# menmitsu/opticalFlowClustering

Measured on AMD Instinct MI355X. Metric: Mpixels/s dense flow+kmeans @1080p, higher is better.
Workload: dtype f32 storage, f64 accumulation; 1 GPU; BASELINE.json configs[2]: 300-frame 1080p synthetic clip, Farneback flow (0.5,3,15,3,5,1.2,0) + Lloyd k=5 over (u,v), frames sharded over 1 GPU(s); width=1920, height=1080, frames=300, pairs=299, k=5, lloyd_iters=11, flow_batch_pairs=64

## Files before the change

### include/ofc.h

```cpp
#ifndef OFC_H
#define OFC_H
#include <stddef.h>
#include <stdint.h>

#ifdef __cplusplus
extern "C" {
#endif

#define OFC_VERSION 100

enum {
    OFC_OK = 0,
    OFC_EINVAL = -1,
    OFC_ENODEV = -2,
    OFC_EHIP = -3,
    OFC_ENOMEM = -4,
    OFC_ENOTREADY = -5,
    OFC_EUNSUPPORTED = -6,
    OFC_ECOMM = -7
};

enum { OFC_U8 = 0, OFC_F32 = 1, OFC_F64 = 2 };

int ofc_version(void);
// ... 67 lines not shown
int ofc_grid_cell_means(int device, const uint8_t *bgr, int W, int H, int rows, int cols,
                        uint8_t *mean_bgr, uint8_t *hsv);

int ofc_kmeans_fit(int device, const void *X, int dtype, int64_t N, int d, int k,
                   const double *init, int max_iter, double tol_rel, double *centers,
                   int32_t *labels, double *inertia, int *n_iter);
int ofc_kmeans_predict(int device, const void *X, int dtype, int64_t N, int d, int k,
                       const double *centers, int32_t *labels);
int ofc_kmeans_fit_dev(int device, const void *X_dev, int dtype, int64_t N, int d, int k,
                       const double *init, int max_iter, double tol_rel, double *centers,
                       uint8_t *labels_dev, double *inertia, int *n_iter);
int ofc_kmeans_fit_dev_stats(int device, const void *X_dev, int dtype, int64_t N, int d, int k,
                             const double *init, int max_iter, double tol_rel, const double *colsum,
                             double *centers, uint8_t *labels_dev, double *inertia, int *n_iter);
int ofc_lloyd_prune_stats(int device, double *out6);
int ofc_bench_lloyd_sweep(int device, const float *X_dev, int64_t N, int k, const double *centers, const double *mean,
                          int what, int iters, float *ms_per_launch);
int ofc_lloyd_colstats_dev(int device, const void *X_dev, int dtype, int64_t N, int d, const double *mean,
                           int pass, double *out);
int ofc_lloyd_step_dev(int device, const void *X_dev, int dtype, int64_t N, int d, int k, const double *mean,
                       const double *centers_c, uint8_t *labels_dev, int accumulate, double *record);
int ofc_lloyd_inertia_dev(int device, const void *X_dev, int dtype, int64_t N, int d, int k, const double *mean,
                          const double *centers_c, const uint8_t *labels_dev, double *inertia);
int ofc_lloyd_farthest_dev(int device, const void *X_dev, int dtype, int64_t N, int d, int k, const double *mean,
                           const double *centers_c, const uint8_t *labels_dev, const int64_t *excl, int n_excl,
                           double *dist2, int64_t *index, double *x_c, int *label);

int ofc_kmeans_fit_w(int device, const void *X, int dtype, const void *w, int w_dtype, int64_t N, int d, int k,
                     const double *init, int max_iter, double tol_rel, double *centers, int32_t *labels,
                     double *inertia, int *n_iter);
// ... 75 lines not shown
```

### opticalflowclustering_amd/_lib.py

```python
import ctypes as C
import os

import numpy as np

_HERE = os.path.dirname(os.path.abspath(__file__))
LIB_PATH = os.path.join(_HERE, "libofc.so")

OFC_OK, OFC_EINVAL, OFC_ENODEV, OFC_EHIP, OFC_ENOMEM, OFC_ENOTREADY, OFC_EUNSUPPORTED, OFC_ECOMM = \
    0, -1, -2, -3, -4, -5, -6, -7
U8, F32, F64 = 0, 1, 2
UNIQUE_ID_BYTES = 128
KPP_CHUNK = 1024


class OfcError(RuntimeError):
    def __init__(self, code, msg):
        super().__init__(f"libofc error {code}: {msg}")
        self.code = code


class FbParams(C.Structure):
    _fields_ = [("pyr_scale", C.c_double), ("levels", C.c_int), ("winsize", C.c_int),
                ("iterations", C.c_int), ("poly_n", C.c_int), ("poly_sigma", C.c_double),
                ("flags", C.c_int)]
# ... 35 lines not shown
    "ofc_flow_resize": ([_i, _vp, _i, _i, _i, _i, _f, _vp], _i),
    "ofc_flow_iterate": ([_i, _vp, _vp, _vp, _i, _i, _i, _i, _i, _i, _vp], _i),
    "ofc_bench_flow_iters": ([_i, _i, _i, _i, _i, _i, C.POINTER(_f)], _i),
    "ofc_bench_polyexp": ([_i, _i, _i, _i, _i, _i, C.POINTER(_f)], _i),
    "ofc_bgr2gray": ([_i, _vp, _i, _i, _vp], _i),
    "ofc_flow_to_bgr": ([_i, _vp, _i, _i, _vp, C.POINTER(_f)], _i),
    "ofc_flow_to_bgr_dev": ([_i, _vp, _i, _i, _i, _vp, _vp], _i),
    "ofc_bgr2hsv": ([_i, _vp, _i64, _vp], _i),
    "ofc_preprocess_rgba": ([_i, _vp, _i64, _i, _vp], _i),
    "ofc_grid_cell_means": ([_i, _vp, _i, _i, _i, _i, _vp, _vp], _i),
    "ofc_kmeans_fit": ([_i, _vp, _i, _i64, _i, _i, _vp, _i, _d, _vp, _vp, C.POINTER(_d), _ip], _i),
    "ofc_kmeans_predict": ([_i, _vp, _i, _i64, _i, _i, _vp, _vp], _i),
    "ofc_kmeans_fit_dev": ([_i, _vp, _i, _i64, _i, _i, _vp, _i, _d, _vp, _vp, C.POINTER(_d), _ip], _i),
    "ofc_kmeans_fit_dev_stats": ([_i, _vp, _i, _i64, _i, _i, _vp, _i, _d, _vp, _vp, _vp, C.POINTER(_d), _ip], _i),
    "ofc_lloyd_prune_stats": ([_i, _vp], _i),
    "ofc_bench_lloyd_sweep": ([_i, _vp, _i64, _i, _vp, _vp, _i, _i, C.POINTER(_f)], _i),
    "ofc_lloyd_colstats_dev": ([_i, _vp, _i, _i64, _i, _vp, _i, _vp], _i),
    "ofc_lloyd_step_dev": ([_i, _vp, _i, _i64, _i, _i, _vp, _vp, _vp, _i, _vp], _i),
    "ofc_lloyd_inertia_dev": ([_i, _vp, _i, _i64, _i, _i, _vp, _vp, _vp, C.POINTER(_d)], _i),
    "ofc_lloyd_farthest_dev": ([_i, _vp, _i, _i64, _i, _i, _vp, _vp, _vp, _vp, _i, C.POINTER(_d), C.POINTER(_i64), _vp, _ip], _i),
    "ofc_kmeans_fit_w": ([_i, _vp, _i, _vp, _i, _i64, _i, _i, _vp, _i, _d, _vp, _vp, C.POINTER(_d), _ip], _i),
    "ofc_kmeans_fit_dev_w": ([_i, _vp, _i, _vp, _i, _i64, _i, _i, _vp, _i, _d, _vp, _vp, _vp, C.POINTER(_d), _ip], _i),
    "ofc_kmeans_score": ([_i, _vp, _i, _vp, _i, _i64, _i, _i, _vp, C.POINTER(_d)], _i),
    "ofc_lloyd_step_dev_w": ([_i, _vp, _i, _vp, _i, _i64, _i, _i, _vp, _vp, _vp, _vp], _i),
    "ofc_lloyd_inertia_dev_w": ([_i, _vp, _i, _vp, _i, _i64, _i, _i, _vp, _vp, _vp, C.POINTER(_d)], _i),
    "ofc_lloyd_farthest_dev_w": ([_i, _vp, _i, _vp, _i, _i64, _i, _i, _vp, _vp, _vp, _vp, _i, C.POINTER(_d), C.POINTER(_i64), _vp, _ip,
                                  C.POINTER(_d)], _i),
    "ofc_flow_weights_dev": ([_i, _vp, _i64, _i, _f, _vp], _i),
    "ofc_bench_lloyd_sweep_w": ([_i, _vp, _vp, _i, _i64, _i, _vp, _vp, _i, C.POINTER(_f)], _i),
    "ofc_kpp_candidates": ([_i, _vp, _i, _i64, _i, _vp, _vp, _i, _vp, _vp, _vp], _i),
# ... 95 lines not shown
```

### opticalflowclustering_amd/cluster.py

```python
import ctypes as C

import numpy as np

from . import _lib
from ._lib import check, load, ptr

_DT = {np.dtype(np.uint8): _lib.U8, np.dtype(np.float32): _lib.F32, np.dtype(np.float64): _lib.F64}


def _as_supported(X):
    X = np.asarray(X)
    if X.ndim != 2:
        raise ValueError(f"Expected 2D array, got {X.ndim}D array instead")
    if X.dtype not in _DT:
        X = X.astype(np.float64)
    return np.ascontiguousarray(X)


def _as_weights(sample_weight, N):
    if sample_weight is None:
        return None
    w = np.asarray(sample_weight)
    if w.ndim == 0:
        w = np.full(N, w, dtype=w.dtype)
# ... 221 lines not shown
        check(load().ofc_kmeans_fit_dev_w(device, C.c_void_p(X_ptr), dtype, C.c_void_p(weights_ptr), weight_dtype, N, d, k, ptr(C0),
                                          max_iter, tol, ptr(cs), ptr(centers), C.c_void_p(labels_ptr) if labels_ptr else None,
                                          C.byref(inertia), C.byref(n_iter)))
        return centers, inertia.value, n_iter.value
    check(load().ofc_kmeans_fit_dev_stats(device, C.c_void_p(X_ptr), dtype, N, d, k, ptr(C0), max_iter, tol, ptr(cs), ptr(centers),
                                          C.c_void_p(labels_ptr) if labels_ptr else None, C.byref(inertia), C.byref(n_iter)))
    return centers, inertia.value, n_iter.value


def prune_stats(device=0):
    out = np.zeros(6, np.float64)
    check(load().ofc_lloyd_prune_stats(device, ptr(out)))
    return {"tile_sweeps": int(out[0]), "pruned_sweeps": int(out[1]), "probe_sweeps": int(out[4]), "final_pruned": bool(out[5]),
            "tiles_tested": int(out[2]), "tiles_pure": int(out[3]),
            "skip_fraction": float(out[3] / out[2]) if out[2] > 0 else 0.0}
```

### opticalflowclustering_amd/csrc/lloyd_api.cpp

```cpp
#include "lloyd_common.h"

#include <algorithm>
#include <cmath>
#include <cstdlib>
#include <mutex>

namespace ofc {

static int lloyd_grid(int64_t N)
{
    return (int)std::max<int64_t>(1, std::min<int64_t>(cdiv64(N / 4, 256), N >= (200ll << 20) ? 2048 : 1024));
}

static size_t dtype_size(int dtype) { return dtype == OFC_U8 ? 1 : (dtype == OFC_F32 ? 4 : 8); }

struct LloydScratch {
    DevBuf state, partial, tot, tot_local, excl, far, labels;
    DevBuf tile_box, tile_sum, tile_sq;
    DevBuf tile_meta;
    DevBuf kpp_closest, kpp_cs, kpp_ss;
    DevBuf kpp_io;
    double prune_stats[6] = {0, 0, 0, 0, 0, 0};
    LloydStatus *status = nullptr;
    LloydStatus *status_dev = nullptr;
    hipStream_t stream = nullptr;
    bool ready = false;
    std::mutex mu;
    int init()
    {
        if (ready) return OFC_OK;
        constexpr int NVMAX = LLOYD_NVMAX;
        OFC_HIP(hipStreamCreateWithFlags(&stream, hipStreamNonBlocking));
        OFC_TRY(state.alloc(sizeof(LloydState)));
        OFC_TRY(partial.alloc(sizeof(double) * 2048 * NVMAX));
        OFC_TRY(tot.alloc(sizeof(double) * (NVMAX + 8)));
        OFC_TRY(tot_local.alloc(sizeof(double) * (NVMAX + 8)));
        OFC_TRY(excl.alloc(sizeof(int64_t) * LLOYD_KMAX));
        OFC_TRY(far.alloc(sizeof(double) * 2 * 2048));
        OFC_TRY(tile_meta.alloc(sizeof(double) * 8));
        OFC_HIP(hipHostMalloc((void **)&status, sizeof(LloydStatus) * LLOYD_WINDOW, hipHostMallocMapped));
        OFC_HIP(hipHostGetDevicePointer((void **)&status_dev, status, 0));
        ready = true;
        return OFC_OK;
    }
};

static int prune_policy_for(int dtype, int64_t N, int d, int k)
{
    if (!lloyd_tiles_supported(dtype, d, k) || N < 64) return LLOYD_PRUNE_OFF;
    const char *e = getenv("OFC_LLOYD_PRUNE");
    const int v = (e && e[0] >= '0' && e[0] <= '3' && !e[1]) ? e[0] - '0' : LLOYD_PRUNE_AUTO;
    if (v == LLOYD_PRUNE_AUTO && N < (1ll << 20)) return LLOYD_PRUNE_OFF;
    return v;
}

static LloydScratch &scratch_for(int device)
{
    static LloydScratch *pool = new LloydScratch[16];
    return pool[device & 15];
}

static int relocate_empty(LloydScratch &sc, const void *X, int dtype, int64_t N, int d, int k, int kmax,
                          int nblocks, const uint8_t *labels, const double *mean_h, const void *wdev = nullptr,
                          int w_dtype = OFC_F32)
{
    hipStream_t s = sc.stream;
    const int NV = lloyd_record_len(kmax, d);
    std::vector<double> tot(NV);
// ... 135 lines not shown
    for (int f = 0; f < d; f++) mean_h[f] = hbuf[f] / Ng;
    OFC_HIP(hipMemcpyAsync(st->mean, mean_h, sizeof(double) * d, hipMemcpyHostToDevice, s));

    double c0[LLOYD_KMAX * LLOYD_DMAX];
    for (int j = 0; j < k * d; j++) c0[j] = init[j] - mean_h[j % d];
    OFC_HIP(hipMemcpyAsync(st->centers, c0, sizeof(double) * k * d, hipMemcpyHostToDevice, s));
    const int prune = wdev ? LLOYD_PRUNE_OFF : prune_policy_for(dtype, N, d, k);
    if (prune) {
        const size_t need = (size_t)(N >> 6) * 16;
        if (sc.tile_box.bytes < need) {
            OFC_TRY(sc.tile_box.alloc(need));
            OFC_TRY(sc.tile_sum.alloc(need));
            OFC_TRY(sc.tile_sq.alloc(need / 2));
        }
    }
    for (double &v : sc.prune_stats) v = 0;
    OFC_TRY(launch_lloyd_set_centers(st, k, d, s, prune));
    bool strict = false, labelled = false, stop = false;
    int tiles_next = LLOYD_TILES_FULL;
    const bool trace = getenv("OFC_LLOYD_TRACE") != nullptr;
    int it = 0;
    const int *halt = &st->halt;
    double *tot_local = dist_has_comm() ? sc.tot_local.as<double>() : tot;
    int window = 4;
    while (it < max_iter && !stop) {
        const int nwin = std::min(window, max_iter - it);
        window = std::min(2 * window, LLOYD_WINDOW);
        for (int w = 0; w < nwin; w++) sc.status[w].valid = 0;
        for (int w = 0; w < nwin; w++) {
            const int tiles = (prune && !labelled) ? (it + w == 0 ? 1 : 2) : 0;
            if (tiles == 1) {
                OFC_TRY(launch_lloyd_tiles((const float *)X, N, k, st, nullptr, nullptr, nullptr, nullptr,
                                           sc.partial.as<double>(), nblocks, LLOYD_WHAT_PROBE, nullptr, s));
                OFC_TRY(launch_lloyd_tiles((const float *)X, N, k, st, sc.tile_box.p, sc.tile_sum.p, sc.tile_sq.p, nullptr,
                                           sc.partial.as<double>(), nblocks, LLOYD_WHAT_META, nullptr, s));
                OFC_TRY(launch_reduce_records(sc.partial.as<double>(), nblocks, 2, sc.tile_meta.as<double>(), s));
            }
            if (tiles)
                OFC_TRY(launch_lloyd_tiles((const float *)X, N, k, st, sc.tile_box.p, sc.tile_sum.p, sc.tile_sq.p, nullptr,
                                           sc.partial.as<double>(), nblocks, LLOYD_WHAT_SWEEP,
                                           tiles == 1 ? sc.tile_meta.as<double>() : nullptr, s));
            else if (wdev)
                OFC_TRY(launch_lloyd_assign_w(X, dtype, wdev, w_dtype, N, d, k, st, labels_dev, sc.partial.as<double>(),
                                              nblocks, labelled ? 1 : 3, it + w == 0, s));
            else
                OFC_TRY(launch_lloyd_assign(X, dtype, N, d, k, st, labels_dev, sc.partial.as<double>(), nblocks,
                                            labelled ? 1 : 3, it + w == 0, s));
            OFC_TRY(launch_reduce_records(sc.partial.as<double>(), nblocks, NV, tot_local, s, halt));
            OFC_TRY(dist_allreduce_f64(tot_local, tot, NV, DIST_SUM, s));
            OFC_TRY(launch_lloyd_update(st, tot, k, d, 0, labelled, it + w == 0, Ng, tol_rel, sc.status_dev + w, s, tiles));
        }
        OFC_HIP(hipStreamSynchronize(s));
        int done = nwin;
        for (int w = 0; w < nwin; w++) {
            LloydStatus &S = sc.status[w];
            if (!S.valid) { set_error("internal: Lloyd iteration %d did not run", it + w); return OFC_EHIP; }
            if (trace)
                fprintf(stderr, "[ofc lloyd] it %d tiles_mode %d tested %.0f pure %.0f shift %.3e empty %d\n", it + w,
                        S.tiles_mode, S.tiles_tested, S.tiles_pure, S.shift_tot, S.n_empty);
            if (S.tiles_mode != -1) {
                tiles_next = S.tiles_next;
                sc.prune_stats[0] += 1;
                if (S.tiles_mode == LLOYD_TILES_PRUNED) {
// ... 20 lines not shown
                OFC_TRY(launch_lloyd_update(st, tot, k, d, 1, was_labelled, it + w == 0, Ng, tol_rel, sc.status_dev + w, s));
                OFC_HIP(hipStreamSynchronize(s));
                done = w + 1;
                if (S.converged) { strict = S.strict != 0; it += w; stop = true; }
                break;
            }
            if (S.converged) { strict = S.strict != 0; it += w; stop = true; break; }
        }
        if (!stop) it += done;
    }
    if (!stop) it = max_iter - 1;
    const bool final_tiles = !strict && prune && !labelled && tiles_next == LLOYD_TILES_PRUNED;
    sc.prune_stats[5] = final_tiles ? 1 : 0;
    if (final_tiles)
        OFC_TRY(launch_lloyd_tiles((const float *)X, N, k, st, sc.tile_box.p, sc.tile_sum.p, sc.tile_sq.p, labels_dev,
                                   sc.partial.as<double>(), nblocks, LLOYD_WHAT_FINAL, nullptr, s));
    else if (!strict && wdev)
        OFC_TRY(launch_lloyd_assign_w(X, dtype, wdev, w_dtype, N, d, k, st, labels_dev, sc.partial.as<double>(), nblocks, 2, 0, s));
    else if (!strict)
        OFC_TRY(launch_lloyd_assign(X, dtype, N, d, k, st, labels_dev, sc.partial.as<double>(), nblocks, 2, 0, s));
    else if (wdev)
        OFC_TRY(launch_lloyd_inertia_w(X, dtype, wdev, w_dtype, N, d, st, labels_dev, sc.partial.as<double>(), nblocks, s));
    else
        OFC_TRY(launch_lloyd_inertia(X, dtype, N, d, st, labels_dev, sc.partial.as<double>(), nblocks, s));
    OFC_TRY(launch_reduce_records(sc.partial.as<double>(), nblocks, 1, tot, s));
    OFC_TRY(dist_allreduce_f64(tot, 1, DIST_SUM, s));
    double in = 0, cfin[LLOYD_KMAX * LLOYD_DMAX];
    OFC_HIP(hipMemcpyAsync(&in, tot, sizeof(double), hipMemcpyDeviceToHost, s));
    OFC_HIP(hipMemcpyAsync(cfin, st->centers, sizeof(double) * k * d, hipMemcpyDeviceToHost, s));
    OFC_HIP(hipStreamSynchronize(s));
    for (int j = 0; j < k * d; j++) centers[j] = cfin[j] + mean_h[j % d];
    if (inertia) *inertia = in;
    if (n_iter) *n_iter = it + 1;
    return OFC_OK;
}

static int lloyd_predict_dev(int device, const void *X, int dtype, int64_t N, int d, int k,
                             const double *centers, uint8_t *labels_dev)
{
    OFC_TRY(ensure_device(device));
// ... 31 lines not shown
    return lloyd_fit_dev(device, X_dev, dtype, N, d, k, init, max_iter, tol_rel, centers, labels_dev, inertia, n_iter);
}

int ofc_bench_lloyd_sweep(int device, const float *X_dev, int64_t N, int k, const double *centers, const double *mean,
                          int what, int iters, float *ms_per_launch)
{
    OFC_REQUIRE(X_dev && centers && mean && ms_per_launch && iters >= 1 && N >= 64, "bad arguments");
    OFC_REQUIRE(what >= 0 && what <= 5, "what = %d outside 0..5", what);
    if (!lloyd_tiles_supported(OFC_F32, 2, k)) { set_error("k=%d outside 1..8", k); return OFC_EUNSUPPORTED; }
    OFC_TRY(ensure_device(device));
    LloydScratch &sc = scratch_for(device);
    std::lock_guard<std::mutex> lock(sc.mu);
    OFC_TRY(sc.init());
    hipStream_t s = sc.stream;
    const int nblocks = lloyd_grid(N);
    const size_t need = (size_t)(N >> 6) * 16;
    if (sc.tile_box.bytes < need) {
        OFC_TRY(sc.tile_box.alloc(need));
        OFC_TRY(sc.tile_sum.alloc(need));
        OFC_TRY(sc.tile_sq.alloc(need / 2));
    }
    if (sc.labels.bytes < (size_t)N) OFC_TRY(sc.labels.alloc((size_t)N));
    LloydState *st = sc.state.as<LloydState>();
    OFC_HIP(hipMemsetAsync(st, 0, sizeof(LloydState), s));
    double c0[LLOYD_KMAX * LLOYD_DMAX];
    for (int j = 0; j < k * 2; j++) c0[j] = centers[j] - mean[j % 2];
    OFC_HIP(hipMemcpyAsync(st->mean, mean, sizeof(double) * 2, hipMemcpyHostToDevice, s));
    OFC_HIP(hipMemcpyAsync(st->centers, c0, sizeof(double) * k * 2, hipMemcpyHostToDevice, s));
    OFC_TRY(launch_lloyd_set_centers(st, k, 2, s, LLOYD_PRUNE_ALWAYS));
    double *partial = sc.partial.as<double>();
    const float *X = X_dev;
    auto launch = [&]() -> int {
        switch (what) {
        case 0: return launch_lloyd_assign(X, OFC_F32, N, 2, k, st, sc.labels.as<uint8_t>(), partial, nblocks, 3, 0, s);
        case 1: case 5: return launch_lloyd_tiles(X, N, k, st, sc.tile_box.p, sc.tile_sum.p, sc.tile_sq.p, nullptr, partial, nblocks, LLOYD_WHAT_SWEEP, nullptr, s);
        case 2: return launch_lloyd_tiles(X, N, k, st, sc.tile_box.p, sc.tile_sum.p, sc.tile_sq.p, nullptr, partial, nblocks, LLOYD_WHAT_META, nullptr, s);
        case 3: return launch_lloyd_assign(X, OFC_F32, N, 2, k, st, sc.labels.as<uint8_t>(), partial, nblocks, 2, 0, s);
        default: return launch_lloyd_tiles(X, N, k, st, sc.tile_box.p, sc.tile_sum.p, sc.tile_sq.p, sc.labels.as<uint8_t>(), partial, nblocks, LLOYD_WHAT_FINAL, nullptr, s);
        }
    };
    if (what == 1 || what == 4 || what == 5) {
        OFC_TRY(launch_lloyd_tiles(X, N, k, st, sc.tile_box.p, sc.tile_sum.p, sc.tile_sq.p, nullptr, partial, nblocks, LLOYD_WHAT_META, nullptr, s));
        const int mode = what == 5 ? LLOYD_TILES_FULL : LLOYD_TILES_PRUNED;
        OFC_HIP(hipMemcpyAsync(&st->prune_mode, &mode, sizeof(int), hipMemcpyHostToDevice, s));
    }
    hipEvent_t e0, e1;
    OFC_HIP(hipEventCreate(&e0));
    OFC_HIP(hipEventCreate(&e1));
    for (int w = 0; w < 2; w++) OFC_TRY(launch());
    OFC_HIP(hipEventRecord(e0, s));
    for (int i = 0; i < iters; i++) OFC_TRY(launch());
    OFC_HIP(hipEventRecord(e1, s));
    OFC_HIP(hipEventSynchronize(e1));
    float ms = 0;
    OFC_HIP(hipEventElapsedTime(&ms, e0, e1));
    *ms_per_launch = ms / iters;
    (void)hipEventDestroy(e0);
    (void)hipEventDestroy(e1);
    return OFC_OK;
}

int ofc_lloyd_prune_stats(int device, double *out6)
{
    OFC_REQUIRE(out6, "null pointer");
    OFC_TRY(ensure_device(device));
    LloydScratch &sc = scratch_for(device);
    std::lock_guard<std::mutex> lock(sc.mu);
    for (int i = 0; i < 6; i++) out6[i] = sc.prune_stats[i];
    return OFC_OK;
}

int ofc_kmeans_fit_dev_stats(int device, const void *X_dev, int dtype, int64_t N, int d, int k, const double *init,
                             int max_iter, double tol_rel, const double *colsum, double *centers, uint8_t *labels_dev,
                             double *inertia, int *n_iter)
// ... 760 lines not shown
```

### opticalflowclustering_amd/csrc/lloyd_common.h

```cpp
#pragma once
#include "ofc_common.h"

#include <cmath>

namespace ofc {

constexpr int LLOYD_KMAX = 16;
constexpr int LLOYD_DMAX = 4;

struct LloydState {
    double mean[LLOYD_DMAX];
    double centers[LLOYD_KMAX * LLOYD_DMAX];
    double centers_new[LLOYD_KMAX * LLOYD_DMAX];
    double cn[LLOYD_KMAX];
    double tol;
    int halt;
    int pad;
    int prune_policy;
    int prune_mode;
    int prune_cooldown, prune_backoff;
};

enum { LLOYD_TILES_FULL = 0,
       LLOYD_TILES_PRUNED = 1,
// ... 15 lines not shown
    int tiles_next;
};

int lloyd_kmax(int k);
int launch_lloyd_colstats(const void *X, int dtype, int64_t N, int d, const double *mean, int pass,
                          double *partial, int nblocks, hipStream_t s);
int launch_reduce_records(const double *partial, int nblocks, int nv, double *out, hipStream_t s,
                          const int *halt = nullptr);
int launch_lloyd_assign(const void *X, int dtype, int64_t N, int d, int k, const LloydState *st,
                        uint8_t *labels, double *partial, int nblocks, int mode, int first, hipStream_t s);
constexpr int LLOYD_REC_EXTRA = 1 + LLOYD_DMAX + 2;
constexpr int LLOYD_NVMAX = LLOYD_KMAX * LLOYD_DMAX + LLOYD_KMAX + LLOYD_REC_EXTRA;
inline int lloyd_record_len(int kmax, int d) { return kmax * d + kmax + LLOYD_REC_EXTRA; }
enum { LLOYD_WHAT_SWEEP = 0, LLOYD_WHAT_META = 1, LLOYD_WHAT_FINAL = 2, LLOYD_WHAT_PROBE = 3 };
bool lloyd_tiles_supported(int dtype, int d, int k);
int launch_lloyd_tiles(const float *X, int64_t N, int k, const LloydState *st, void *box, void *tsum, void *tsq,
                       uint8_t *labels, double *partial, int nblocks, int what, const double *meta, hipStream_t s);
int launch_lloyd_update(LloydState *st, const double *tot, int k, int d, int after_reloc, int labelled, int first,
                        double n_total, double tol_rel, LloydStatus *status, hipStream_t s, int tiles = 0);
constexpr int LLOYD_WINDOW = 16;
int launch_lloyd_set_centers(LloydState *st, int k, int d, hipStream_t s, int prune_policy = 0);
int launch_lloyd_inertia(const void *X, int dtype, int64_t N, int d, const LloydState *st,
                         const uint8_t *labels, double *partial, int nblocks, hipStream_t s);
int launch_grid_assign_counts(const float *flow, const LloydState *st, int W, int H, int n_frames, int rows, int cols, int k,
                              int32_t *counts, double *sums, hipStream_t s);
inline int check_uv_model(int k, const double *mean, const double *centers_c)
{
    OFC_REQUIRE(centers_c, "null pointer");
    if (k < 1 || k > LLOYD_KMAX) {
        set_error("k=%d outside the kernel's range (1..%d)", k, LLOYD_KMAX);
// ... 56 lines not shown
```

### opticalflowclustering_amd/csrc/lloyd_tiles.hip

```cpp
#include "lloyd_common.h"

#include <algorithm>

namespace ofc {

typedef float v4f __attribute__((ext_vector_type(4)));
typedef double v2d __attribute__((ext_vector_type(2)));

template <int N> __device__ __forceinline__ int row_ror(int v)
{
    return __builtin_amdgcn_update_dpp(0, v, 0x120 + N, 0xf, 0xf, false);
}
template <int N> __device__ __forceinline__ float row_ror(float v) { return __int_as_float(row_ror<N>(__float_as_int(v))); }
template <int N> __device__ __forceinline__ double row_ror(double v)
{
    return __hiloint2double(row_ror<N>(__double2hiint(v)), row_ror<N>(__double2loint(v)));
}
__device__ __forceinline__ float row_min(float v)
{
    v = fminf(v, row_ror<8>(v)); v = fminf(v, row_ror<4>(v)); v = fminf(v, row_ror<2>(v)); return fminf(v, row_ror<1>(v));
}
__device__ __forceinline__ float row_max(float v)
{
    v = fmaxf(v, row_ror<8>(v)); v = fmaxf(v, row_ror<4>(v)); v = fmaxf(v, row_ror<2>(v)); return fmaxf(v, row_ror<1>(v));
// ... 184 lines not shown
        sq0 += x0 * x0;
        sq1 += x1 * x1;
    }
    for (int off = 32; off >= 1; off >>= 1) {
        sq0 += __shfl_down(sq0, off, 64);
        sq1 += __shfl_down(sq1, off, 64);
    }
    if (lane == 0) { s_red[wave][0] = sq0; s_red[wave][1] = sq1; }
    __syncthreads();
    if (tid < 2) partial[(size_t)blockIdx.x * 2 + tid] = ((s_red[0][tid] + s_red[1][tid]) + s_red[2][tid]) + s_red[3][tid];
}

enum { TILES_SWEEP = 0, TILES_FINAL = 1 };

template <int KMAX, int WHAT>
__global__ __launch_bounds__(256) void k_lloyd_tiles(const float *__restrict__ X, int64_t N,
                                                     const LloydState *__restrict__ st, const v4f *__restrict__ box,
                                                     const v2d *__restrict__ tsum, const double *__restrict__ tsq,
                                                     uint8_t *__restrict__ labels, double *__restrict__ partial,
                                                     const double *__restrict__ meta)
{
    constexpr int D = 2, k = KMAX;
    constexpr int NV = KMAX * D + KMAX + LLOYD_REC_EXTRA;
    constexpr bool FINAL = WHAT == TILES_FINAL, ACCUM = !FINAL;
    if (ACCUM && st->halt) return;
    const int mode = ACCUM ? st->prune_mode : LLOYD_TILES_PRUNED;
    const bool own_sq = ACCUM && meta && st->prune_policy == LLOYD_PRUNE_OFF;
    double sq0 = 0, sq1 = 0;
    extern __shared__ __align__(16) unsigned char smem[];
    double *sacc = reinterpret_cast<double *>(smem);
    unsigned *scnt = reinterpret_cast<unsigned *>(sacc + (size_t)k * D * 256);
    __shared__ unsigned s_tiles[4][2];
    __shared__ double s_cen[KMAX][4];
    const int tid = threadIdx.x, lane = tid & 63, wave = tid >> 6, row = lane >> 4, r16 = lane & 15;
    if (ACCUM) {
        for (int i = 0; i < k * D; i++) sacc[i * 256 + tid] = 0.0;
        for (int j = 0; j < k; j++) scnt[j * 256 + tid] = 0u;
    }
    TileCtx<KMAX> cx;
    cx.load(st, s_cen);
    double inert = 0;
    unsigned n_tested = 0, n_pure = 0;
    auto accumulate = [&](int l, double x0, double x1, unsigned n) {
        sacc[(l * D) * 256 + tid] += x0;
        sacc[(l * D + 1) * 256 + tid] += x1;
        scnt[l * 256 + tid] += n;
    };
    auto walk = [&](int64_t t, const v4f a, const v4f b) {
        double x[4][D];
// ... 16 lines not shown
                    sq1 += x[p][1] * x[p][1];
                }
            }
        }
        if (FINAL) {
#pragma unroll
            for (int p = 0; p < 4; p++) inert += cx.sq_dist(x[p][0], x[p][1], nl[p]);
            __builtin_nontemporal_store((unsigned)(nl[0] | (nl[1] << 8) | (nl[2] << 16) | (nl[3] << 24)),
                                        reinterpret_cast<unsigned *>(labels) + t * 16 + r16);
        }
    };

    const int64_t NT = N >> 6;
    const int64_t NG = (NT + 63) >> 6;
    const int64_t wg = (int64_t)blockIdx.x * 4 + wave, nw = (int64_t)gridDim.x * 4;
    for (int64_t g = wg; g < NG; g += nw) {
        const int64_t t = g * 64 + lane;
        const bool valid = t < NT;
        unsigned long long todo;
        if (mode == LLOYD_TILES_FULL) {
            todo = __ballot(valid);
        } else {
            int j = -1;
            if (valid) {
                const v4f b = box[t];
                j = cx.box_label((double)b.x - cx.m[0], (double)b.y - cx.m[1], (double)b.z - cx.m[0], (double)b.w - cx.m[1]);
                n_tested += 1u;
                n_pure += (j >= 0);
            }
            const bool skip = j >= 0 && mode == LLOYD_TILES_PRUNED;
            if (skip) {
                const v2d s = tsum[t];
                if (ACCUM) accumulate(j, s.x, s.y, 64u);
                if (FINAL) {
#pragma clang fp contract(off)
                    double cjx, cjy, cnj;
                    cx.centre_of(j, cjx, cjy, cnj);
                    const double du = s.x * 0.015625 - cjx, dv = s.y * 0.015625 - cjy;
                    inert += tsq[t] + 64.0 * (du * du + dv * dv);
                    const unsigned w4 = (unsigned)j * 0x01010101u;
                    typedef unsigned v4u __attribute__((ext_vector_type(4)));
                    v4u *lp = reinterpret_cast<v4u *>(labels + t * 64);
#pragma unroll
                    for (int q = 0; q < 4; q++) __builtin_nontemporal_store((v4u){w4, w4, w4, w4}, lp + q);
                }
            }
            todo = __ballot(valid && !skip);
        }
        while (todo) {
            int ta[8];
#pragma unroll
            for (int i = 0; i < 8; i++) {
                if (todo) {
                    ta[i] = __builtin_ctzll(todo);
                    todo &= todo - 1;
                } else {
                    ta[i] = -1;
                }
            }
            const int tA = row == 0 ? ta[0] : row == 1 ? ta[1] : row == 2 ? ta[2] : ta[3];
            const int tB = row == 0 ? ta[4] : row == 1 ? ta[5] : row == 2 ? ta[6] : ta[7];
            const int64_t tileA = g * 64 + tA, tileB = g * 64 + tB;
            v4f a0 = {0, 0, 0, 0}, a1 = a0, b0 = a0, b1 = a0;
            if (tA >= 0) {
                const v4f *p = reinterpret_cast<const v4f *>(X + tileA * 128 + r16 * 8);
                a0 = __builtin_nontemporal_load(p);
                a1 = __builtin_nontemporal_load(p + 1);
            }
            if (tB >= 0) {
                const v4f *p = reinterpret_cast<const v4f *>(X + tileB * 128 + r16 * 8);
                b0 = __builtin_nontemporal_load(p);
                b1 = __builtin_nontemporal_load(p + 1);
            }
            if (tA >= 0) walk(tileA, a0, a1);
            if (tB >= 0) walk(tileB, b0, b1);
        }
    }
    if (blockIdx.x == 0 && tid < (int)(N - NT * 64)) {
        const int64_t i = NT * 64 + tid;
        const double x0 = (double)X[i * 2] - cx.m[0], x1 = (double)X[i * 2 + 1] - cx.m[1];
        const int l = cx.label_of(x0, x1);
        if (ACCUM) accumulate(l, x0, x1, 1u);
        if (own_sq) {
            sq0 += x0 * x0;
            sq1 += x1 * x1;
        }
        if (FINAL) {
            inert += cx.sq_dist(x0, x1, l);
            labels[i] = (uint8_t)l;
        }
    }
    if (FINAL) {
// ... 32 lines not shown
        __shared__ double lds_sq[4][2];
        for (int off = 32; off >= 1; off >>= 1) {
            sq0 += __shfl_down(sq0, off, 64);
            sq1 += __shfl_down(sq1, off, 64);
        }
        if (lane == 0) { lds_sq[wave][0] = sq0; lds_sq[wave][1] = sq1; }
        __syncthreads();
        if (tid < D) rec[KMAX * D + KMAX + 1 + tid] = ((lds_sq[0][tid] + lds_sq[1][tid]) + lds_sq[2][tid]) + lds_sq[3][tid];
    } else if (meta && blockIdx.x == 0 && tid >= 64 && tid < 64 + D) {
        rec[KMAX * D + KMAX + 1 + (tid - 64)] = meta[tid - 64];
    }
}

bool lloyd_tiles_supported(int dtype, int d, int k) { return dtype == OFC_F32 && d == 2 && k >= 1 && k <= 8; }

template <int KMAX>
static void launch_tiles_k(const float *X, int64_t N, const LloydState *st, void *box, void *tsum, void *tsq, uint8_t *labels,
                           double *partial, int nblocks, int what, const double *meta, hipStream_t s)
{
    const size_t lds = (size_t)KMAX * (8 * 2 + 4) * 256;
    v4f *b = (v4f *)box;
    v2d *ts = (v2d *)tsum;
    double *tq = (double *)tsq;
    if (what == LLOYD_WHAT_PROBE) {
        const int pb = std::min(nblocks, 256);
        hipLaunchKernelGGL((k_tile_probe<KMAX>), dim3(pb), dim3(256), 0, s, X, N, st, partial);
        hipLaunchKernelGGL(k_tile_decide, dim3(1), dim3(64), 0, s, const_cast<LloydState *>(st), partial, pb);
    } else if (what == LLOYD_WHAT_META)
        hipLaunchKernelGGL(k_tile_meta, dim3(nblocks), dim3(256), 0, s, X, N, st, b, ts, tq, partial);
    else if (what == LLOYD_WHAT_FINAL)
        hipLaunchKernelGGL((k_lloyd_tiles<KMAX, TILES_FINAL>), dim3(nblocks), dim3(256), 0, s, X, N, st, b, ts, tq, labels, partial, nullptr);
    else
        hipLaunchKernelGGL((k_lloyd_tiles<KMAX, TILES_SWEEP>), dim3(nblocks), dim3(256), lds, s, X, N, st, b, ts, tq, labels, partial, meta);
}

// ... 20 lines not shown
```

Before: 17150 Mpixels/s.

## Size tile-sweep grids by occupancy and prefetch tile metadata across sweep iterations

Tile kernels (probe, meta, sweep, final) now get grid sizes computed per kernel from HIP occupancy queries times CU count, capped by tile count and an env override, instead of one shared block count. The sweep loop is restructured so box and sum metadata for the next tile group is fetched while the current group is processed, and point loads are issued before the walk of the previous pair. Label stores for pure tiles move after the walk with lane shuffles, and launch bounds add a minimum-occupancy hint. The aim is better latency hiding and a grid better matched to the hardware, at the cost of extra registers and more complex control flow.

```diff
diff --git a/include/ofc.h b/include/ofc.h
--- a/include/ofc.h
+++ b/include/ofc.h
@@ -105,6 +105,7 @@
                              const double *init, int max_iter, double tol_rel, const double *colsum,
                              double *centers, uint8_t *labels_dev, double *inertia, int *n_iter);
 int ofc_lloyd_prune_stats(int device, double *out6);
+int ofc_lloyd_tiles_grid(int device, int what, int k, int64_t N, int *blocks, int *resident_per_cu);
 int ofc_bench_lloyd_sweep(int device, const float *X_dev, int64_t N, int k, const double *centers, const double *mean,
                           int what, int iters, float *ms_per_launch);
 int ofc_lloyd_colstats_dev(int device, const void *X_dev, int dtype, int64_t N, int d, const double *mean,
diff --git a/opticalflowclustering_amd/_lib.py b/opticalflowclustering_amd/_lib.py
--- a/opticalflowclustering_amd/_lib.py
+++ b/opticalflowclustering_amd/_lib.py
@@ -73,6 +73,7 @@
     "ofc_kmeans_fit_dev": ([_i, _vp, _i, _i64, _i, _i, _vp, _i, _d, _vp, _vp, C.POINTER(_d), _ip], _i),
     "ofc_kmeans_fit_dev_stats": ([_i, _vp, _i, _i64, _i, _i, _vp, _i, _d, _vp, _vp, _vp, C.POINTER(_d), _ip], _i),
     "ofc_lloyd_prune_stats": ([_i, _vp], _i),
+    "ofc_lloyd_tiles_grid": ([_i, _i, _i, _i64, _ip, _ip], _i),
     "ofc_bench_lloyd_sweep": ([_i, _vp, _i64, _i, _vp, _vp, _i, _i, C.POINTER(_f)], _i),
     "ofc_lloyd_colstats_dev": ([_i, _vp, _i, _i64, _i, _vp, _i, _vp], _i),
     "ofc_lloyd_step_dev": ([_i, _vp, _i, _i64, _i, _i, _vp, _vp, _vp, _i, _vp], _i),
diff --git a/opticalflowclustering_amd/cluster.py b/opticalflowclustering_amd/cluster.py
--- a/opticalflowclustering_amd/cluster.py
+++ b/opticalflowclustering_amd/cluster.py
@@ -259,3 +259,12 @@
     return {"tile_sweeps": int(out[0]), "pruned_sweeps": int(out[1]), "probe_sweeps": int(out[4]), "final_pruned": bool(out[5]),
             "tiles_tested": int(out[2]), "tiles_pure": int(out[3]),
             "skip_fraction": float(out[3] / out[2]) if out[2] > 0 else 0.0}
+
+
+TILES_SWEEP, TILES_META, TILES_FINAL, TILES_PROBE = 0, 1, 2, 3
+
+
+def lloyd_tiles_grid(what, k, N, device=0):
+    blocks, resident = C.c_int(), C.c_int()
+    check(load().ofc_lloyd_tiles_grid(device, what, k, N, C.byref(blocks), C.byref(resident)))
+    return blocks.value, resident.value
diff --git a/opticalflowclustering_amd/csrc/lloyd_api.cpp b/opticalflowclustering_amd/csrc/lloyd_api.cpp
--- a/opticalflowclustering_amd/csrc/lloyd_api.cpp
+++ b/opticalflowclustering_amd/csrc/lloyd_api.cpp
@@ -32,11 +32,11 @@
         constexpr int NVMAX = LLOYD_NVMAX;
         OFC_HIP(hipStreamCreateWithFlags(&stream, hipStreamNonBlocking));
         OFC_TRY(state.alloc(sizeof(LloydState)));
-        OFC_TRY(partial.alloc(sizeof(double) * 2048 * NVMAX));
+        OFC_TRY(partial.alloc(sizeof(double) * LLOYD_GRID_MAX * NVMAX));
         OFC_TRY(tot.alloc(sizeof(double) * (NVMAX + 8)));
         OFC_TRY(tot_local.alloc(sizeof(double) * (NVMAX + 8)));
         OFC_TRY(excl.alloc(sizeof(int64_t) * LLOYD_KMAX));
-        OFC_TRY(far.alloc(sizeof(double) * 2 * 2048));
+        OFC_TRY(far.alloc(sizeof(double) * 2 * LLOYD_GRID_MAX));
         OFC_TRY(tile_meta.alloc(sizeof(double) * 8));
         OFC_HIP(hipHostMalloc((void **)&status, sizeof(LloydStatus) * LLOYD_WINDOW, hipHostMallocMapped));
         OFC_HIP(hipHostGetDevicePointer((void **)&status_dev, status, 0));
@@ -52,6 +52,21 @@
     const int v = (e && e[0] >= '0' && e[0] <= '3' && !e[1]) ? e[0] - '0' : LLOYD_PRUNE_AUTO;
     if (v == LLOYD_PRUNE_AUTO && N < (1ll << 20)) return LLOYD_PRUNE_OFF;
     return v;
+}
+
+static int tile_blocks(int device, int what, int k, int64_t N, int *blocks, int *resident_per_cu = nullptr)
+{
+    long cap = LLOYD_GRID_MAX;
+    const char *e = getenv("OFC_LLOYD_GRID");
+    if (e && e[0]) {
+        char *end = nullptr;
+        cap = strtol(e, &end, 10);
+        OFC_REQUIRE(!*end && cap >= 1 && cap <= LLOYD_GRID_MAX, "OFC_LLOYD_GRID=%s is not a work-group count in 1..%d", e,
+                    LLOYD_GRID_MAX);
+    }
+    OFC_TRY(lloyd_tiles_grid(device, what, k, N, blocks, resident_per_cu));
+    *blocks = (int)std::min<long>(*blocks, cap);
+    return OFC_OK;
 }
 
 static LloydScratch &scratch_for(int device)
@@ -217,6 +232,13 @@
             OFC_TRY(sc.tile_sq.alloc(need / 2));
         }
     }
+    int nb_probe = 1, nb_meta = 1, nb_sweep = 1, nb_final = 1;
+    if (prune) {
+        OFC_TRY(tile_blocks(device, LLOYD_WHAT_PROBE, k, N, &nb_probe));
+        OFC_TRY(tile_blocks(device, LLOYD_WHAT_META, k, N, &nb_meta));
+        OFC_TRY(tile_blocks(device, LLOYD_WHAT_SWEEP, k, N, &nb_sweep));
+        OFC_TRY(tile_blocks(device, LLOYD_WHAT_FINAL, k, N, &nb_final));
+    }
     for (double &v : sc.prune_stats) v = 0;
     OFC_TRY(launch_lloyd_set_centers(st, k, d, s, prune));
     bool strict = false, labelled = false, stop = false;
@@ -234,14 +256,14 @@
             const int tiles = (prune && !labelled) ? (it + w == 0 ? 1 : 2) : 0;
             if (tiles == 1) {
                 OFC_TRY(launch_lloyd_tiles((const float *)X, N, k, st, nullptr, nullptr, nullptr, nullptr,
-                                           sc.partial.as<double>(), nblocks, LLOYD_WHAT_PROBE, nullptr, s));
+                                           sc.partial.as<double>(), nb_probe, LLOYD_WHAT_PROBE, nullptr, s));
                 OFC_TRY(launch_lloyd_tiles((const float *)X, N, k, st, sc.tile_box.p, sc.tile_sum.p, sc.tile_sq.p, nullptr,
-                                           sc.partial.as<double>(), nblocks, LLOYD_WHAT_META, nullptr, s));
-                OFC_TRY(launch_reduce_records(sc.partial.as<double>(), nblocks, 2, sc.tile_meta.as<double>(), s));
+                                           sc.partial.as<double>(), nb_meta, LLOYD_WHAT_META, nullptr, s));
+                OFC_TRY(launch_reduce_records(sc.partial.as<double>(), nb_meta, 2, sc.tile_meta.as<double>(), s));
             }
             if (tiles)
                 OFC_TRY(launch_lloyd_tiles((const float *)X, N, k, st, sc.tile_box.p, sc.tile_sum.p, sc.tile_sq.p, nullptr,
-                                           sc.partial.as<double>(), nblocks, LLOYD_WHAT_SWEEP,
+                                           sc.partial.as<double>(), nb_sweep, LLOYD_WHAT_SWEEP,
                                            tiles == 1 ? sc.tile_meta.as<double>() : nullptr, s));
             else if (wdev)
                 OFC_TRY(launch_lloyd_assign_w(X, dtype, wdev, w_dtype, N, d, k, st, labels_dev, sc.partial.as<double>(),
@@ -249,7 +271,7 @@
             else
                 OFC_TRY(launch_lloyd_assign(X, dtype, N, d, k, st, labels_dev, sc.partial.as<double>(), nblocks,
                                             labelled ? 1 : 3, it + w == 0, s));
-            OFC_TRY(launch_reduce_records(sc.partial.as<double>(), nblocks, NV, tot_local, s, halt));
+            OFC_TRY(launch_reduce_records(sc.partial.as<double>(), tiles ? nb_sweep : nblocks, NV, tot_local, s, halt));
             OFC_TRY(dist_allreduce_f64(tot_local, tot, NV, DIST_SUM, s));
             OFC_TRY(launch_lloyd_update(st, tot, k, d, 0, labelled, it + w == 0, Ng, tol_rel, sc.status_dev + w, s, tiles));
         }
@@ -300,7 +322,7 @@
     sc.prune_stats[5] = final_tiles ? 1 : 0;
     if (final_tiles)
         OFC_TRY(launch_lloyd_tiles((const float *)X, N, k, st, sc.tile_box.p, sc.tile_sum.p, sc.tile_sq.p, labels_dev,
-                                   sc.partial.as<double>(), nblocks, LLOYD_WHAT_FINAL, nullptr, s));
+                                   sc.partial.as<double>(), nb_final, LLOYD_WHAT_FINAL, nullptr, s));
     else if (!strict && wdev)
         OFC_TRY(launch_lloyd_assign_w(X, dtype, wdev, w_dtype, N, d, k, st, labels_dev, sc.partial.as<double>(), nblocks, 2, 0, s));
     else if (!strict)
@@ -309,7 +331,7 @@
         OFC_TRY(launch_lloyd_inertia_w(X, dtype, wdev, w_dtype, N, d, st, labels_dev, sc.partial.as<double>(), nblocks, s));
     else
         OFC_TRY(launch_lloyd_inertia(X, dtype, N, d, st, labels_dev, sc.partial.as<double>(), nblocks, s));
-    OFC_TRY(launch_reduce_records(sc.partial.as<double>(), nblocks, 1, tot, s));
+    OFC_TRY(launch_reduce_records(sc.partial.as<double>(), final_tiles ? nb_final : nblocks, 1, tot, s));
     OFC_TRY(dist_allreduce_f64(tot, 1, DIST_SUM, s));
     double in = 0, cfin[LLOYD_KMAX * LLOYD_DMAX];
     OFC_HIP(hipMemcpyAsync(&in, tot, sizeof(double), hipMemcpyDeviceToHost, s));
@@ -371,6 +393,10 @@
     OFC_TRY(sc.init());
     hipStream_t s = sc.stream;
     const int nblocks = lloyd_grid(N);
+    int nb_meta, nb_sweep, nb_final;
+    OFC_TRY(tile_blocks(device, LLOYD_WHAT_META, k, N, &nb_meta));
+    OFC_TRY(tile_blocks(device, LLOYD_WHAT_SWEEP, k, N, &nb_sweep));
+    OFC_TRY(tile_blocks(device, LLOYD_WHAT_FINAL, k, N, &nb_final));
     const size_t need = (size_t)(N >> 6) * 16;
     if (sc.tile_box.bytes < need) {
         OFC_TRY(sc.tile_box.alloc(need));
@@ -390,14 +416,14 @@
     auto launch = [&]() -> int {
         switch (what) {
         case 0: return launch_lloyd_assign(X, OFC_F32, N, 2, k, st, sc.labels.as<uint8_t>(), partial, nblocks, 3, 0, s);
-        case 1: case 5: return launch_lloyd_tiles(X, N, k, st, sc.tile_box.p, sc.tile_sum.p, sc.tile_sq.p, nullptr, partial, nblocks, LLOYD_WHAT_SWEEP, nullptr, s);
-        case 2: return launch_lloyd_tiles(X, N, k, st, sc.tile_box.p, sc.tile_sum.p, sc.tile_sq.p, nullptr, partial, nblocks, LLOYD_WHAT_META, nullptr, s);
+        case 1: case 5: return launch_lloyd_tiles(X, N, k, st, sc.tile_box.p, sc.tile_sum.p, sc.tile_sq.p, nullptr, partial, nb_sweep, LLOYD_WHAT_SWEEP, nullptr, s);
+        case 2: return launch_lloyd_tiles(X, N, k, st, sc.tile_box.p, sc.tile_sum.p, sc.tile_sq.p, nullptr, partial, nb_meta, LLOYD_WHAT_META, nullptr, s);
         case 3: return launch_lloyd_assign(X, OFC_F32, N, 2, k, st, sc.labels.as<uint8_t>(), partial, nblocks, 2, 0, s);
-        default: return launch_lloyd_tiles(X, N, k, st, sc.tile_box.p, sc.tile_sum.p, sc.tile_sq.p, sc.labels.as<uint8_t>(), partial, nblocks, LLOYD_WHAT_FINAL, nullptr, s);
+        default: return launch_lloyd_tiles(X, N, k, st, sc.tile_box.p, sc.tile_sum.p, sc.tile_sq.p, sc.labels.as<uint8_t>(), partial, nb_final, LLOYD_WHAT_FINAL, nullptr, s);
         }
     };
     if (what == 1 || what == 4 || what == 5) {
-        OFC_TRY(launch_lloyd_tiles(X, N, k, st, sc.tile_box.p, sc.tile_sum.p, sc.tile_sq.p, nullptr, partial, nblocks, LLOYD_WHAT_META, nullptr, s));
+        OFC_TRY(launch_lloyd_tiles(X, N, k, st, sc.tile_box.p, sc.tile_sum.p, sc.tile_sq.p, nullptr, partial, nb_meta, LLOYD_WHAT_META, nullptr, s));
         const int mode = what == 5 ? LLOYD_TILES_FULL : LLOYD_TILES_PRUNED;
         OFC_HIP(hipMemcpyAsync(&st->prune_mode, &mode, sizeof(int), hipMemcpyHostToDevice, s));
     }
@@ -415,6 +441,13 @@
     (void)hipEventDestroy(e0);
     (void)hipEventDestroy(e1);
     return OFC_OK;
+}
+
+int ofc_lloyd_tiles_grid(int device, int what, int k, int64_t N, int *blocks, int *resident_per_cu)
+{
+    OFC_REQUIRE(blocks && resident_per_cu, "null pointer");
+    OFC_TRY(ensure_device(device));
+    return tile_blocks(device, what, k, N, blocks, resident_per_cu);
 }
 
 int ofc_lloyd_prune_stats(int device, double *out6)
diff --git a/opticalflowclustering_amd/csrc/lloyd_common.h b/opticalflowclustering_amd/csrc/lloyd_common.h
--- a/opticalflowclustering_amd/csrc/lloyd_common.h
+++ b/opticalflowclustering_amd/csrc/lloyd_common.h
@@ -53,6 +53,8 @@
 inline int lloyd_record_len(int kmax, int d) { return kmax * d + kmax + LLOYD_REC_EXTRA; }
 enum { LLOYD_WHAT_SWEEP = 0, LLOYD_WHAT_META = 1, LLOYD_WHAT_FINAL = 2, LLOYD_WHAT_PROBE = 3 };
 bool lloyd_tiles_supported(int dtype, int d, int k);
+constexpr int LLOYD_GRID_MAX = 2048;
+int lloyd_tiles_grid(int device, int what, int k, int64_t N, int *blocks, int *resident_per_cu);
 int launch_lloyd_tiles(const float *X, int64_t N, int k, const LloydState *st, void *box, void *tsum, void *tsq,
                        uint8_t *labels, double *partial, int nblocks, int what, const double *meta, hipStream_t s);
 int launch_lloyd_update(LloydState *st, const double *tot, int k, int d, int after_reloc, int labelled, int first,
diff --git a/opticalflowclustering_amd/csrc/lloyd_tiles.hip b/opticalflowclustering_amd/csrc/lloyd_tiles.hip
--- a/opticalflowclustering_amd/csrc/lloyd_tiles.hip
+++ b/opticalflowclustering_amd/csrc/lloyd_tiles.hip
@@ -1,6 +1,8 @@
 #include "lloyd_common.h"
 
 #include <algorithm>
+#include <mutex>
+#include <type_traits>
 
 namespace ofc {
 
@@ -222,7 +224,7 @@
 enum { TILES_SWEEP = 0, TILES_FINAL = 1 };
 
 template <int KMAX, int WHAT>
-__global__ __launch_bounds__(256) void k_lloyd_tiles(const float *__restrict__ X, int64_t N,
+__global__ __launch_bounds__(256, WHAT == TILES_FINAL ? 8 : 6) void k_lloyd_tiles(const float *__restrict__ X, int64_t N,
                                                      const LloydState *__restrict__ st, const v4f *__restrict__ box,
                                                      const v2d *__restrict__ tsum, const double *__restrict__ tsq,
                                                      uint8_t *__restrict__ labels, double *__restrict__ partial,
@@ -240,7 +242,8 @@
     unsigned *scnt = reinterpret_cast<unsigned *>(sacc + (size_t)k * D * 256);
     __shared__ unsigned s_tiles[4][2];
     __shared__ double s_cen[KMAX][4];
-    const int tid = threadIdx.x, lane = tid & 63, wave = tid >> 6, row = lane >> 4, r16 = lane & 15;
+    const int tid = threadIdx.x, lane = tid & 63, row = lane >> 4, r16 = lane & 15;
+    const int wave = __builtin_amdgcn_readfirstlane(tid >> 6);
     if (ACCUM) {
         for (int i = 0; i < k * D; i++) sacc[i * 256 + tid] = 0.0;
         for (int j = 0; j < k; j++) scnt[j * 256 + tid] = 0u;
@@ -287,40 +290,19 @@
     const int64_t NT = N >> 6;
     const int64_t NG = (NT + 63) >> 6;
     const int64_t wg = (int64_t)blockIdx.x * 4 + wave, nw = (int64_t)gridDim.x * 4;
-    for (int64_t g = wg; g < NG; g += nw) {
-        const int64_t t = g * 64 + lane;
-        const bool valid = t < NT;
-        unsigned long long todo;
-        if (mode == LLOYD_TILES_FULL) {
-            todo = __ballot(valid);
-        } else {
-            int j = -1;
-            if (valid) {
-                const v4f b = box[t];
-                j = cx.box_label((double)b.x - cx.m[0], (double)b.y - cx.m[1], (double)b.z - cx.m[0], (double)b.w - cx.m[1]);
-                n_tested += 1u;
-                n_pure += (j >= 0);
-            }
-            const bool skip = j >= 0 && mode == LLOYD_TILES_PRUNED;
-            if (skip) {
-                const v2d s = tsum[t];
-                if (ACCUM) accumulate(j, s.x, s.y, 64u);
-                if (FINAL) {
-#pragma clang fp contract(off)
-                    double cjx, cjy, cnj;
-                    cx.centre_of(j, cjx, cjy, cnj);
-                    const double du = s.x * 0.015625 - cjx, dv = s.y * 0.015625 - cjy;
-                    inert += tsq[t] + 64.0 * (du * du + dv * dv);
-                    const unsigned w4 = (unsigned)j * 0x01010101u;
-                    typedef unsigned v4u __attribute__((ext_vector_type(4)));
-                    v4u *lp = reinterpret_cast<v4u *>(labels + t * 64);
-#pragma unroll
-                    for (int q = 0; q < 4; q++) __builtin_nontemporal_store((v4u){w4, w4, w4, w4}, lp + q);
-                }
-            }
-            todo = __ballot(valid && !skip);
-        }
-        while (todo) {
+    auto sweep = [&](auto tested_c) {
+        constexpr bool TESTED = decltype(tested_c)::value;
+        v4f nbox = {0, 0, 0, 0};
+        v2d nsum = {0, 0};
+        auto fetch_meta = [&](int64_t g) {
+            if (!TESTED) return;
+            const int64_t t = g < NG ? std::min<int64_t>(g * 64 + lane, NT - 1) : NT - 1;
+            nbox = box[t];
+            if (ACCUM) nsum = tsum[t];
+        };
+        int tA = -1, tB = -1;
+        v4f a0 = {0, 0, 0, 0}, a1 = a0, b0 = a0, b1 = a0;
+        auto request = [&](int64_t g, unsigned long long &todo) {
             int ta[8];
 #pragma unroll
             for (int i = 0; i < 8; i++) {
@@ -331,24 +313,74 @@
                     ta[i] = -1;
                 }
             }
-            const int tA = row == 0 ? ta[0] : row == 1 ? ta[1] : row == 2 ? ta[2] : ta[3];
-            const int tB = row == 0 ? ta[4] : row == 1 ? ta[5] : row == 2 ? ta[6] : ta[7];
-            const int64_t tileA = g * 64 + tA, tileB = g * 64 + tB;
-            v4f a0 = {0, 0, 0, 0}, a1 = a0, b0 = a0, b1 = a0;
+            tA = row == 0 ? ta[0] : row == 1 ? ta[1] : row == 2 ? ta[2] : ta[3];
+            tB = row == 0 ? ta[4] : row == 1 ? ta[5] : row == 2 ? ta[6] : ta[7];
+            a0 = a1 = b0 = b1 = v4f{0, 0, 0, 0};
             if (tA >= 0) {
-                const v4f *p = reinterpret_cast<const v4f *>(X + tileA * 128 + r16 * 8);
+                const v4f *p = reinterpret_cast<const v4f *>(X + (g * 64 + tA) * 128 + r16 * 8);
                 a0 = __builtin_nontemporal_load(p);
                 a1 = __builtin_nontemporal_load(p + 1);
             }
             if (tB >= 0) {
-                const v4f *p = reinterpret_cast<const v4f *>(X + tileB * 128 + r16 * 8);
+                const v4f *p = reinterpret_cast<const v4f *>(X + (g * 64 + tB) * 128 + r16 * 8);
                 b0 = __builtin_nontemporal_load(p);
                 b1 = __builtin_nontemporal_load(p + 1);
             }
-            if (tA >= 0) walk(tileA, a0, a1);
-            if (tB >= 0) walk(tileB, b0, b1);
-        }
-    }
+        };
+        if (wg < NG) fetch_meta(wg);
+        for (int64_t g = wg; g < NG; g += nw) {
+            const int64_t t = g * 64 + lane;
+            const bool valid = t < NT;
+            v2d s = nsum;
+            int j = -1;
+            if (TESTED && valid) {
+                const v4f b = nbox;
+                j = cx.box_label((double)b.x - cx.m[0], (double)b.y - cx.m[1], (double)b.z - cx.m[0], (double)b.w - cx.m[1]);
+                n_tested += 1u;
+                n_pure += (j >= 0);
+            }
+            const bool skip = j >= 0 && mode == LLOYD_TILES_PRUNED;
+            unsigned long long todo = __ballot(valid && !skip);
+            request(g, todo);
+            double sq = 0;
+            if (FINAL) {
+                const int64_t tc = std::min<int64_t>(t, NT - 1);
+                s = tsum[tc];
+                sq = tsq[tc];
+            }
+            fetch_meta(g + nw);
+            if (skip) {
+                if (ACCUM) accumulate(j, s.x, s.y, 64u);
+                if (FINAL) {
+#pragma clang fp contract(off)
+                    double cjx, cjy, cnj;
+                    cx.centre_of(j, cjx, cjy, cnj);
+                    const double du = s.x * 0.015625 - cjx, dv = s.y * 0.015625 - cjy;
+                    inert += sq + 64.0 * (du * du + dv * dv);
+                }
+            }
+            for (;;) {
+                if (tA >= 0) walk(g * 64 + tA, a0, a1);
+                if (tB >= 0) walk(g * 64 + tB, b0, b1);
+                if (!todo) break;
+                request(g, todo);
+            }
+            if (FINAL) {
+                __builtin_amdgcn_s_waitcnt(0x0f70);
+                typedef unsigned v4u __attribute__((ext_vector_type(4)));
+                const int verdict = skip ? j : -1;
+                v4u *lp = reinterpret_cast<v4u *>(labels + g * 4096) + lane;
+#pragma unroll
+                for (int q = 0; q < 4; q++) {
+                    const int jq = __shfl(verdict, 16 * q + (lane >> 2), 64);
+                    const unsigned w4 = (unsigned)jq * 0x01010101u;
+                    if (jq >= 0) __builtin_nontemporal_store((v4u){w4, w4, w4, w4}, lp + q * 64);
+                }
+            }
+        }
+    };
+    if (mode != LLOYD_TILES_FULL) sweep(std::true_type{});
+    else sweep(std::false_type{});
     if (blockIdx.x == 0 && tid < (int)(N - NT * 64)) {
         const int64_t i = NT * 64 + tid;
         const double x0 = (double)X[i * 2] - cx.m[0], x1 = (double)X[i * 2 + 1] - cx.m[1];
@@ -411,11 +443,63 @@
 
 bool lloyd_tiles_supported(int dtype, int d, int k) { return dtype == OFC_F32 && d == 2 && k >= 1 && k <= 8; }
 
+template <int KMAX> constexpr size_t sweep_lds() { return (size_t)KMAX * (8 * 2 + 4) * 256; }
+
+template <int KMAX> static hipError_t resident_k(int what, int *n)
+{
+    switch (what) {
+    case LLOYD_WHAT_PROBE: return hipOccupancyMaxActiveBlocksPerMultiprocessor(n, k_tile_probe<KMAX>, 256, 0);
+    case LLOYD_WHAT_META: return hipOccupancyMaxActiveBlocksPerMultiprocessor(n, k_tile_meta, 256, 0);
+    case LLOYD_WHAT_FINAL: return hipOccupancyMaxActiveBlocksPerMultiprocessor(n, k_lloyd_tiles<KMAX, TILES_FINAL>, 256, 0);
+    default: return hipOccupancyMaxActiveBlocksPerMultiprocessor(n, k_lloyd_tiles<KMAX, TILES_SWEEP>, 256, sweep_lds<KMAX>());
+    }
+}
+
+int lloyd_tiles_grid(int device, int what, int k, int64_t N, int *blocks, int *resident_per_cu)
+{
+    static std::mutex mu;
+    static int cache[16][4][8], cus[16];
+    OFC_REQUIRE(what >= LLOYD_WHAT_SWEEP && what <= LLOYD_WHAT_PROBE, "what = %d outside 0..3", what);
+    OFC_REQUIRE(device >= 0 && device < 16 && N >= 0 && blocks, "bad arguments");
+    if (k < 1 || k > 8) { set_error("k=%d outside the tile sweep's range (1..8)", k); return OFC_EUNSUPPORTED; }
+    int res, ncu;
+    {
+        std::lock_guard<std::mutex> lock(mu);
+        int &slot = cache[device][what][k - 1];
+        if (!slot) {
+            int n = 0;
+            hipError_t e = hipErrorInvalidValue;
+            switch (k) {
+            case 1: e = resident_k<1>(what, &n); break;
+            case 2: e = resident_k<2>(what, &n); break;
+            case 3: e = resident_k<3>(what, &n); break;
+            case 4: e = resident_k<4>(what, &n); break;
+            case 5: e = resident_k<5>(what, &n); break;
+            case 6: e = resident_k<6>(what, &n); break;
+            case 7: e = resident_k<7>(what, &n); break;
+            case 8: e = resident_k<8>(what, &n); break;
+            }
+            OFC_HIP(e);
+            OFC_HIP(hipDeviceGetAttribute(&cus[device], hipDeviceAttributeMultiprocessorCount, device));
+            slot = std::max(n, 1);
+        }
+        res = slot;
+        ncu = std::max(cus[device], 1);
+    }
+    const int64_t NT = N >> 6;
+    const int64_t waves = what == LLOYD_WHAT_META || what == LLOYD_WHAT_PROBE ? (NT + 3) >> 2 : (NT + 63) >> 6;
+    int64_t nb = std::min<int64_t>((int64_t)res * ncu, (waves + 3) >> 2);
+    nb = std::min<int64_t>(nb, what == LLOYD_WHAT_PROBE ? 256 : LLOYD_GRID_MAX);
+    *blocks = (int)std::max<int64_t>(nb, 1);
+    if (resident_per_cu) *resident_per_cu = res;
+    return OFC_OK;
+}
+
 template <int KMAX>
 static void launch_tiles_k(const float *X, int64_t N, const LloydState *st, void *box, void *tsum, void *tsq, uint8_t *labels,
                            double *partial, int nblocks, int what, const double *meta, hipStream_t s)
 {
-    const size_t lds = (size_t)KMAX * (8 * 2 + 4) * 256;
+    const size_t lds = sweep_lds<KMAX>();
     v4f *b = (v4f *)box;
     v2d *ts = (v2d *)tsum;
     double *tq = (double *)tsq;
```

Result: no change. 17310 Mpixels/s, median of 6 (+0.9%).
